# termuxinator/html5-canvas-raytracer

Measured on AMD Instinct MI355X. Metric: Mpixel/s, higher is better.
Workload: dtype f64; 1 GPU; cfg3: h8 scene (8 spheres, 2 lights, depth 3, supersample 1) at 3840x2160; SCENE, CAMERA AND LAUNCH TABLE RESIDENT (a static frame rendered again and again: cold_frame / new_camera_every_step are the other cases); one launch per frame; kernel=fma

## Files before the change

html5-canvas-raytracer_amd/csrc/rt_kernel_trace.h:

```cpp

#define RT_PIN() asm volatile("")
#define RT_ROOT(TCA, DISC)                                                                    \
        const double thc_ = rt_sqrt_nn<REFRACT>(DISC);                                                 \
        const double t0_ = (TCA) - thc_, t1_ = (TCA) + thc_;                                  \
        const bool in_ = (t0_ < eps);                                                         \
        const double t_ = in_ ? t1_ : t0_;
#define RT_CAND(IDX, TCA, DISC)                                                               \
      if (!((DISC) < 0.0)) {                                                                  \
        RT_PIN();                                                                             \
        RT_ROOT(TCA, DISC)                                                                    \
        const bool closer_ = (t_ < ht) && !(t_ < eps);              \
        ht = closer_ ? t_ : ht;                                                               \
        hcode = closer_ ? ((int)(2u * (IDX)) + (in_ ? 1 : 0)) : hcode;                        \
      }
#define RT_GENERIC(IDX, G)                                                                    \
      {                                                                                       \
        const v3 Lv_ = mk((G).ox - p.x, (G).oy - p.y, (G).oz - p.z);                          \
        const double tca_ = dot(d, Lv_);                                                      \
        const double disc_ = (G).r2 - (dot(Lv_, Lv_) - tca_ * tca_);                          \
        RT_CAND(IDX, tca_, disc_)                                                             \
      }
#define RT_ANCHORED_DISC(G)                                                                   \
        const double tca_ = d.x * (G).ox + d.y * (G).oy + d.z * (G).oz;                       \
        const double disc_ = __builtin_fma(tca_, tca_, -(G).r2);
#define RT_ANCHORED(IDX, G)                                                                   \
      {                                                                                       \
        RT_ANCHORED_DISC(G)                                                                   \
        RT_CAND(IDX, tca_, disc_)                                                             \
      }

#if !RT_STRICT
__device__ __forceinline__ float rt_q_of(float qp, float x, float c, float rp_over_r) {
  const float ic = __builtin_amdgcn_rcpf(fmaxf(c, 1e-30f));
  return fminf(ic * (qp * (6.f * x + rp_over_r) + x + 0.5f * x * x) + x, 1e30f);
}
__device__ __forceinline__ int rt_lvl(int lv) { return lv & 255; }
#define RT_Q_GET(L_) __builtin_bit_cast(float, (uint32_t)(L_) & 0xffff0000u)
__device__ __forceinline__ int rt_q_put(int lv, float q) { return (int)(((uint32_t)lv & 0xffffu) | ((__builtin_bit_cast(uint32_t, q) + 0xffffu) & 0xffff0000u)); }
__device__ __forceinline__ float rt_r_get(int lv) { return __builtin_bit_cast(float, ((uint32_t)lv & 0xff00u) << 15); }
__device__ __forceinline__ int rt_r_put(int lv, float r) { return (int)(((uint32_t)lv & 0xffff00ffu) | ((((__builtin_bit_cast(uint32_t, r) >> 23) + 1u) & 255u) << 8)); }
constexpr float RT_Q_FLAT = 4096.f;
#define RT_Q_OF(QP, T, INVR, C, RP) rt_q_of((QP), (T) * (INVR), (C), (RP) * (INVR))
#else
__device__ __forceinline__ int rt_lvl(int lv) { return lv; }
#endif

#if !RT_STRICT
#define RT_XY_INDEX(XU, XV, FU, FV)                                                                                \
          const unsigned long long su = __builtin_bit_cast(unsigned long long, (XU) + 6442450944.0), sv = __builtin_bit_cast(unsigned long long, (XV) + 6442450944.0);   \
          uint32_t iu = __builtin_amdgcn_alignbit((uint32_t)(su >> 32), (uint32_t)su, 20u) ^ 0x80000000u;        \
          uint32_t iv = __builtin_amdgcn_alignbit((uint32_t)(sv >> 32), (uint32_t)sv, 20u) ^ 0x80000000u;       \
           \
          const bool near_ = (min(((uint32_t)su + 1u) & 0xfffffu, ((uint32_t)sv + 1u) & 0xfffffu) <= 2u);           \
           \
          if constexpr (UNI) { if (__ballot(near_) != 0ull) return false; }                                    \
          if (!UNI && near_) {                                                                                  \
            RT_PIN();                                                                                             \
            iu = (uint32_t)(XU); iv = (uint32_t)(XV);                    \
            const rt_launch __attribute__((address_space(4))) *K = rt_cold_args();                                \
             \
            float q_here = RT_Q_GET(level);                                                                        \
            if (rt_lvl(level) == 0 && q_here == 0.f) {                   \
              const float ex = (float)(h.x - K->cam_origin[0]), ey = (float)(h.y - K->cam_origin[1]), ez = (float)(h.z - K->cam_origin[2]);   \
              q_here = RT_Q_OF(0.f, __builtin_sqrtf(ex * ex + ey * ey + ez * ez), (float)m.inv_r, __builtin_fabsf((float)dot(d, n)), 0.f);       \
            }                                                                                                     \
            double tol = (K->mark_flags & RT_MARK_ALL) ? 2.0 : K->flag_tol * (double)fmaxf(1.f, q_here * (1.f / RT_Q_FLAT));   \
                          \
            if ((K->mark_flags & (RT_MARK_WEIGHT | RT_MARK_ALL)) == RT_MARK_WEIGHT) {                              \
              double S_ = map_valid ? acc[0] : 1.0;                                                               \
              if constexpr (FOLD_FORWARD && REFRACT) for (int i_ = 0; i_ < sp; i_++) S_ *= (parked[i_].map_valid ? parked[i_].S : 1.0) * parked[i_].a3;   \
              if (__builtin_fabs(S_) * 510.0 < 0.9) tol = -1.0;                                                    \
            }                                                                                                     \
             \
            const bool zf = !(K->mark_flags & RT_MARK_ZERO);                                                       \
            const bool bu = (zf && (FU) == 0.0 && (XU) == 0.0) || (__builtin_fabs((XU) - __builtin_rint(XU)) >= tol);    \
            const bool bv = (zf && (FV) == 0.0 && (XV) == 0.0) || (__builtin_fabs((XV) - __builtin_rint(XV)) >= tol);    \
            if (!(bu & bv)) {                                                                                      \
              uint32_t t3 = threadIdx.x;                                                                          \
              if constexpr (W1 && !GRID) t3 = rt_lane_again(); else                                               \
              asm volatile("" : "+v"(t3));                                                                        \
              rt_mark_append<SS2>(rt_pixel_of<SS2, W1>(L, t3));                                                        \
            }                                                                                                     \
          }
#endif

#if !RT_STRICT
#define RT_SDISC(G, TC, DISC)                                                                 \
            const double TC = -(sv.x * (G).ox + sv.y * (G).oy + sv.z * (G).oz);               \
            const double DISC = __builtin_fma(TC, TC, -(G).r2);
#define RT_SROOTS(TC, THC, T0, T1) const double T0 = llen - (TC + THC), T1 = llen - (TC - THC);
#else
#define RT_SDISC(G, TC, DISC)                                                                 \
            const v3 Lv_ = mk((G).ox - h.x, (G).oy - h.y, (G).oz - h.z);                      \
            const double TC = dot(sv, Lv_);                                                   \
            const double DISC = (G).r2 - (dot(Lv_, Lv_) - TC * TC);
#define RT_SROOTS(TC, THC, T0, T1) const double T0 = TC - THC, T1 = TC + THC;
#endif
#define RT_SHADOW(J, G)                                                                       \
            {                                                                                 \
              const bool other_ = ((int)(J) != hi);                                           \
              if (COUNT && other_ && !blocked) tests++;                                       \
              RT_SDISC(G, tc_, disc_)                                                         \
              if (other_ && !(disc_ < 0.0) && !blocked) {                                     \
                RT_PIN();                                                                     \
                const double thc_ = rt_sqrt_nn<REFRACT>(disc_);                                        \
                RT_SROOTS(tc_, thc_, t0_, t1_)                                                \
                const double t_ = (t0_ < eps) ? t1_ : t0_;                                    \
                if ((t_ < llen) && !(t_ < eps)) {                                             \
                  RT_PIN();                                                                   \
                  const double oa4_ = objs[J].albedo[4];                                      \
                  if (oa4_ != 0.0) li = rt_div(li, oa4_);    \
                  else { li = 0.0; blocked = true; }                                          \
                }                                                                             \
              }                                                                               \
            }
#define RT_SHADOW_U(J, G)                                                                     \
            {                                                                               \
              RT_SDISC(G, tc_, disc_)                                                       \
              if (((int)(J) != hi) && !(disc_ < 0.0)) {                                     \
                RT_PIN();                                                                   \
                const double thc_ = rt_sqrt_nn<REFRACT>(disc_);                                      \
                RT_SROOTS(tc_, thc_, t0_, t1_)                                              \
                const double t_ = (t0_ < eps) ? t1_ : t0_;                                  \
                if ((t_ < llen) && !(t_ < eps) && li != 0.0) {                              \
                  RT_PIN();                                                                 \
                  const double oa4_ = objs[J].albedo[4];                                    \
                  li = (oa4_ != 0.0) ? rt_div(li, oa4_) : 0.0;                              \
                }                                                                           \
              }                                                                             \
            }

template <bool REFRACT, bool COUNT, bool GRID, bool SS2, bool ITEM = false, bool W1 = false, bool UNI = false>
__device__ __forceinline__ bool trace_pixel(const rt_launch &L, const rt_mtl *mtl, const rt_texture_desc *tex,
                                            [[maybe_unused]] double *acc, [[maybe_unused]] const rt_geom *cull_lds, [[maybe_unused]] const rt_geom cull0, [[maybe_unused]] uint32_t lane,
                                            [[maybe_unused]] double blk_x0, [[maybe_unused]] double blk_x1, [[maybe_unused]] double blk_y0,
                                            [[maybe_unused]] double blk_y1, v3 p, v3 d, double rgb[3], uint32_t cnt[3],
                                            [[maybe_unused]] bool is_probe, [[maybe_unused]] uint32_t cand_host,
                                            [[maybe_unused]] uint32_t own_sx = 0u, [[maybe_unused]] uint32_t own_sy = 0u, [[maybe_unused]] uint32_t own_f = 0u) {
  static_assert(!UNI || (W1 && !REFRACT && !COUNT && !ITEM && !RT_STRICT), "uniform-material path: the one-wave-workgroup product kernels");
#ifdef RT_TESTING
  uint32_t probe_n = 0;
  double probe_li = 0.0;
#endif
  const sphere_kptr objs = (sphere_kptr)L.objects;
  const geom_kptr geom = (geom_kptr)L.geom;
  const uint32_t N = L.n_objects, NL = L.n_lights;
  const double eps = L.epsilon;
  const uint32_t NLOOP = L.n_loop;
  const uint32_t enc = L.enclosing;
  const bool cull_lds_on = (!RT_STRICT && !COUNT) ? (!GRID && !W1) : (L.cull_in_lds != 0u);
#if RT_STRICT
  constexpr bool FOLD_FORWARD = false;
#else
  constexpr bool FOLD_FORWARD = true;
#endif
  constexpr bool LEAN = !RT_STRICT && !REFRACT && !COUNT && !ITEM;
  [[maybe_unused]] frame<REFRACT> stack[FOLD_FORWARD ? 1 : RT_MAX_SEGS];
  [[maybe_unused]] park parked[(FOLD_FORWARD && REFRACT) ? RT_MAX_SEGS : 1];
  [[maybe_unused]] int sp = 0;
  [[maybe_unused]] bool map_valid = false;
  int level = 0;
  [[maybe_unused]] uint32_t tree_path = 1u;
#if defined(RT_TESTING) && defined(RT_ABLATE_BOUNCE)
  uint32_t segs_left = L.segs ? 1 : 0;
#else
  uint32_t segs_left = L.segs;
#endif
  double ret[3] = {0.0, 0.0, 0.0};
  constexpr bool PARK_RET = FOLD_FORWARD && W1 && !GRID && !REFRACT && !COUNT && !ITEM && !UNI;

  double ht = RT_INF; int hcode = -1;
  if constexpr (UNI) { if (segs_left == 0) return false; }
  if (segs_left != 0) {
        [[maybe_unused]] const geom_kptr ga = (geom_kptr)L.geom_cam;
#if !RT_STRICT
        if constexpr (UNI) {
          const uint32_t i = cand_host & 255u;
          const rt_geom g0 = rt_load_geom32(ga, i);
          typename rt_mtl_src<true>::type &mu = *rt_mtl_at<true>(mtl, i);
          if ((mu.albedo[3] > 0.0 && segs_left > 1) || rt_mtl_kind(mu) == RT_SAMPLER_STARS) return false;
          RT_ANCHORED_DISC(g0)
          const double t0_ = tca_ - rt_sqrt_nn<REFRACT>(disc_);
          const bool met_ = !(disc_ < 0.0) && (t0_ < ht) && !(t0_ < eps);
          if (__ballot(!met_) != 0ull) return false;
#if defined(RT_TESTING) && defined(RT_ABLATE_UNIFORM)
          rgb[0] = rgb[1] = rgb[2] = 0.0;
          return true;
#endif
          ht = t0_; hcode = (int)(2u * i);
        } else
        if (cand_host != 0u) {
          { const uint32_t i = cand_host & 255u; const rt_geom g0 = rt_load_geom32(ga, i); RT_ANCHORED(i, g0) }
          if (cand_host >= (2u << 16)) { const uint32_t i = (cand_host >> 8) & 255u; const rt_geom g0 = rt_load_geom32(ga, i); RT_ANCHORED(i, g0) }
        } else
#endif
        for (uint32_t base = 0; base < NLOOP; base += 64u) {
          const uint32_t j = base + lane;
          const uint32_t jj = j < NLOOP ? j : 0u;
          double c0 = cull0.ox, c1 = cull0.oy, c2 = cull0.oz, c3 = cull0.r2;
          if constexpr (ITEM) {
          } else if (cull_lds_on) {
            const rt_geom __attribute__((address_space(3))) *g = (const rt_geom __attribute__((address_space(3))) *)cull_lds + jj;
            c0 = g->ox; c1 = g->oy; c2 = g->oz; c3 = g->r2;
          } else if (base != 0u || (W1 && !GRID)) {
            const rt_geom __attribute__((address_space(1))) *g = (const rt_geom __attribute__((address_space(1))) *)L.cull + jj;
            c0 = g->ox; c1 = g->oy; c2 = g->oz; c3 = g->r2;
          }
          const rt_geom cr = rt_geom{c0, c1, c2, c3};
          unsigned long long m = __ballot(j < NLOOP) & __ballot(cr.ox * L.proj_d <= blk_x1) & __ballot(cr.oy * L.proj_d >= blk_x0) &
                                 __ballot(cr.oz * L.proj_d <= blk_y1) & __ballot(cr.r2 * L.proj_d >= blk_y0);
          if constexpr (ITEM) m = (NLOOP - base >= 64u) ? ~0ull : ((1ull << (NLOOP - base)) - 1ull);
          while (m) {
            const uint32_t i = base + (uint32_t)__builtin_ctzll(m);
            m &= m - 1ull;
#if RT_STRICT
            const rt_geom g0 = rt_load_geom32(geom, i);
            RT_GENERIC(i, g0)
#else
            const rt_geom g0 = rt_load_geom32(ga, i);
            RT_ANCHORED(i, g0)
#endif
          }
        }
  }
  bool searched = true;
  [[maybe_unused]] bool first_bounce = false;
#if !RT_STRICT
  if (!UNI && L.sky_fast && segs_left != 0 && __ballot(hcode >= 0) == 0ull) {
    if (COUNT) { cnt[0]++; cnt[2] += N; }
    rgb[0] = L.sky_rgb[0]; rgb[1] = L.sky_rgb[1]; rgb[2] = L.sky_rgb[2];
    return true;
  }
#endif

  if (segs_left != 0) {
    for (;;) {
      if constexpr (PARK_RET) ret[0] = ret[1] = ret[2] = 0.0;
      if (COUNT) cnt[0]++;
      if (!UNI && !searched) {
        bool scanned = false;
#if !RT_STRICT
        if constexpr (GRID) {
          if (rt_cold_args()->bounce_table != nullptr) {
            const uint32_t from = (uint32_t)(hcode >> 1);
            const double ax = __builtin_fabs(d.x), ay = __builtin_fabs(d.y), az = __builtin_fabs(d.z);
            const bool bx = (ax >= ay) && (ax >= az), by = !bx && (ay >= az);
            const double dm = bx ? d.x : (by ? d.y : d.z);
            const double du = bx ? d.y : d.x, dv = (bx || by) ? d.z : d.y;
            const double sc = (0.5 * RT_BGRID) * __builtin_amdgcn_rcp(__builtin_fabs(dm));
            const double fu = __builtin_fmin(__builtin_fmax(__builtin_fma(du, sc, 0.5 * RT_BGRID), 0.0), (double)(RT_BGRID - 1u));
            const double fv = __builtin_fmin(__builtin_fmax(__builtin_fma(dv, sc, 0.5 * RT_BGRID), 0.0), (double)(RT_BGRID - 1u));
            const uint32_t face = (bx ? 0u : (by ? 2u : 4u)) + ((dm < 0.0) ? 1u : 0u);
            const uint32_t key = from * RT_BCELLS + face * (RT_BGRID * RT_BGRID) + (uint32_t)fv * RT_BGRID + (uint32_t)fu;
            const uint32_t words = (NLOOP + 63u) >> 6;
            ht = RT_INF; hcode = -1;
            for (uint32_t wd = 0; wd < words; wd++) {
              unsigned long long cand = 0ull, todo = __ballot(true);
              uint32_t distinct = 0;
              while (todo) {
                const uint32_t k0 = (uint32_t)__builtin_amdgcn_readlane((int)key, (int)__builtin_ctzll(todo));
                cand |= rt_load_word32(rt_cold_args()->bounce_table, k0 * words + wd);
                todo &= ~__ballot(key == k0);
                if (++distinct == 16u && todo) {
                  cand = (wd + 1u == words && (NLOOP & 63u)) ? ((1ull << (NLOOP & 63u)) - 1ull) : ~0ull;
                  break;
                }
              }
              while (cand) {
                const uint32_t j = (wd << 6) + (uint32_t)__builtin_ctzll(cand);
                cand &= cand - 1ull;
                const rt_geom g0 = rt_load_geom32(geom, j);
                RT_GENERIC(j, g0)
              }
            }
            scanned = true;
          }
        }
#endif
#if !RT_STRICT
        if constexpr (!GRID && !REFRACT && !COUNT && !ITEM) {
          if (first_bounce) {
            uint32_t fb = rt_entry_first_bounce<W1>(L);
#ifdef RT_TESTING
            if (L.no_first_bounce) fb = 0u;
#endif
            if (fb >> 31) {
              ht = RT_INF; hcode = -1;
              uint32_t m = (fb >> RT_CELL_SHIFT) & ((1u << RT_FB_MAX_LOOP) - 1u);
              uint32_t sn = rt_entry_second_node<W1>(L);
#ifdef RT_TESTING
              if (L.no_second_node) sn = 0u;
              if ((sn & (RT_SN_SELF0 | RT_SN_SELF1)) && L.uniform_waves != nullptr && __builtin_ctzll(__ballot(true)) == (int)lane) atomicAdd(L.uniform_waves + 3, 1ull);
#endif
              if (sn & RT_SN_SELF0) m &= ~(1u << (fb & 255u));
              if (sn & RT_SN_SELF1) m &= ~(1u << ((fb >> 8) & 255u));
              while (m) {
                const uint32_t i = (uint32_t)__builtin_ctz(m);
                m &= m - 1u;
                const rt_geom g0 = rt_load_geom32(geom, i);
                RT_GENERIC(i, g0)
              }
              scanned = true;
#ifdef RT_TESTING
              if (L.uniform_waves != nullptr && __builtin_ctzll(__ballot(true)) == (int)lane) atomicAdd(L.uniform_waves + 2, 1ull);
#endif
            }
          }
        }
#endif
        if (!scanned) {
          ht = RT_INF; hcode = -1;
          uint32_t i = 0;
          for (; i + 2 <= NLOOP; i += 2) {
            const rt_geom_pair gp = rt_load_geom_pair32(geom, i);
            const rt_geom g0 = gp.a, g1 = gp.b;
            RT_GENERIC(i, g0) RT_GENERIC(i + 1, g1)
          }
          if (i < NLOOP) { const rt_geom g0 = rt_load_geom32(geom, i); RT_GENERIC(i, g0) }
        }
      }
      [[maybe_unused]] const bool primary_node = UNI || searched;
      first_bounce = searched;
      searched = false;
      if (!UNI && enc != ~0u && hcode < 0) {
        if (L.enclosing_flat) {
          ht = 1.0; hcode = (int)(2u * enc + 1u);
        } else {
          const rt_geom g0 = rt_load_geom32(geom, enc);
          RT_GENERIC(enc, g0)
        }
      }
      if (COUNT) cnt[2] += N;
      const int hi = UNI ? (int)(cand_host & 255u) : (hcode >> 1);
      const bool inside = (hcode & 1) != 0;
      bool descend = false;
#if defined(RT_TESTING) && defined(RT_ABLATE_SHADE)
      if (true) { ret[0] = ht; ret[1] = (double)hcode; ret[2] = 0.0; } else
#endif
      if (!UNI && hcode < 0) {
        { const auto &mc = RT_COLD(miss_color); ret[0] = mc[0]; ret[1] = mc[1]; ret[2] = mc[2]; }
#ifdef RT_TESTING
        if (is_probe && probe_n < RT_PROBE_NODES) {
          double *q = L.probe + (size_t)(probe_n++) * RT_PROBE_WORDS;
          for (uint32_t z = 0; z < RT_PROBE_WORDS; z++) q[z] = 0.0;
          q[0] = (double)(REFRACT ? tree_path : (1u << rt_lvl(level))); q[1] = -1.0; q[2] = ht; q[9] = d.x; q[10] = d.y; q[11] = d.z;
          q[17] = (double)segs_left; q[19] = p.x; q[20] = p.y; q[21] = p.z; q[23] = 1.0;
        }
#endif
      } else {
        typename rt_mtl_src<UNI>::type &m = *rt_mtl_at<UNI>(mtl, (uint32_t)hi);
        const v3 h = mk(p.x + d.x * ht, p.y + d.y * ht, p.z + d.z * ht);
#if RT_STRICT
        double nlen;
        const v3 n = unit(mk(h.x - m.origin[0], h.y - m.origin[1], h.z - m.origin[2]), &nlen);
#else
        const double inv_r = m.inv_r;
        const v3 n = mk((h.x - m.origin[0]) * inv_r, (h.y - m.origin[1]) * inv_r, (h.z - m.origin[2]) * inv_r);
#endif
        v3 l;
        if constexpr (UNI) l = n;
        else l = inside ? mk(-n.x, -n.y, -n.z) : n;
        double a0 = m.albedo[0];
        const double a1 = m.albedo[1], a2 = m.albedo[2];
        double a3 = m.albedo[3];
        const double a4 = REFRACT ? m.albedo[4] : 0.0;
#if !RT_STRICT && !defined(RT_ABLATE_QAMP)
        if (!UNI && (rt_lvl(level) != 0 || ((a3 > 0.0 || a4 > 0.0) && segs_left > 1))) {
          const float ir_ = (float)inv_r;
          const float q_ = RT_Q_OF(RT_Q_GET(level), (float)ht, ir_, __builtin_fabsf((float)dot(d, n)), rt_r_get(level));
          level = rt_q_put(level, q_);
          level = rt_r_put(level, __builtin_amdgcn_rcpf(ir_));
        }
#endif

        double col[3];
#if defined(RT_TESTING) && defined(RT_ABLATE_SAMPLER)
        const int kind = RT_SAMPLER_COLOR;
#else
        const int kind = rt_mtl_kind(m);
#endif
#if RT_STRICT
        if (kind == RT_SAMPLER_TEXTURE) {
          double t_at, t_as;
          rt_atan2_asin<REFRACT>(-n.z, -n.x, -n.y, &t_at, &t_as);
          const double u = RT_DIV_CONST(t_at, M_PI) / 2.0 + 0.5;
          const double v = RT_DIV_CONST(t_as, M_PI / 2.0) / 2.0 + 0.5;
          const rt_texture_desc td = rt_tex_desc<UNI>(tex, rt_mtl_texture(m));
          const double xd = ceil(u * (double)td.width) - 1.0, yd = ceil(v * (double)td.height) - 1.0;
          uint32_t xi = (xd > 0.0) ? (uint32_t)xd : 0u, yi = (yd > 0.0) ? (uint32_t)yd : 0u;
          xi = min(xi, td.width - 1u); yi = min(yi, td.height - 1u);
          const uint32_t texel = *(const uint32_t *)(L.texel_base + td.texels_offset + ((size_t)yi * td.width + xi) * 4u);
          col[0] = RT_DIV_CONST((double)(texel & 255u), 255.0); col[1] = RT_DIV_CONST((double)((texel >> 8) & 255u), 255.0);
          col[2] = RT_DIV_CONST((double)((texel >> 16) & 255u), 255.0);
          if (xd != xd || yd != yd) col[0] = col[1] = col[2] = __builtin_nan("");
        } else if (kind == RT_SAMPLER_CHECKER) {
          double t_at, t_as;
          rt_atan2_asin<REFRACT>(-n.y, -n.x, -n.z, &t_at, &t_as);
          const double u = RT_DIV_CONST(t_at, M_PI) / 2.0 + 0.5;
          const double v = RT_DIV_CONST(t_as, M_PI / 2.0) / 2.0 + 0.5;
          const int c = to_int32_bit0(u * m.c[6]) ^ to_int32_bit0(v * m.c[7]);
          col[0] = m.c[3 * c]; col[1] = m.c[3 * c + 1]; col[2] = m.c[3 * c + 2];
#else
        [[maybe_unused]] double t_at, t_as;
        [[maybe_unused]] const bool one_cell = UNI && !GRID && kind == RT_SAMPLER_CHECKER && (cand_host & (1u << 24)) != 0u;
        if (UNI && one_cell) {
          const uint32_t c3 = (cand_host >> 28) & 1u ? 3u : 0u;
          col[0] = m.c[c3]; col[1] = m.c[c3 + 1u]; col[2] = m.c[c3 + 2u];
        } else if (UNI && kind != RT_SAMPLER_TEXTURE && kind != RT_SAMPLER_CHECKER) {
          col[0] = m.c[0]; col[1] = m.c[1]; col[2] = m.c[2];
        } else {
        if constexpr (UNI) {
          const bool tx_ = (kind == RT_SAMPLER_TEXTURE);
          rt_atan2_asin<REFRACT>(tx_ ? -n.z : -n.y, -n.x, tx_ ? -n.y : -n.z, &t_at, &t_as);
        }
        if (kind == RT_SAMPLER_TEXTURE) {
          if constexpr (!UNI) rt_atan2_asin<REFRACT>(-n.z, -n.x, -n.y, &t_at, &t_as);
          const double u = RT_DIV_CONST(t_at, M_PI) / 2.0 + 0.5;
          const double v = RT_DIV_CONST(t_as, M_PI / 2.0) / 2.0 + 0.5;
          const rt_texture_desc td = rt_tex_desc<UNI>(tex, rt_mtl_texture(m));
          const double xu = u * (double)td.width, xv = v * (double)td.height;
          RT_XY_INDEX(xu, xv, 1.0, 1.0)
          const uint32_t xi = min(iu, td.width - 1u), yi = min(iv, td.height - 1u);
          const uint32_t texel = *(const uint32_t *)(rt_cold_args()->texel_base + td.texels_offset + ((size_t)yi * td.width + xi) * 4u);
          col[0] = RT_DIV_CONST((double)(texel & 255u), 255.0); col[1] = RT_DIV_CONST((double)((texel >> 8) & 255u), 255.0);
          col[2] = RT_DIV_CONST((double)((texel >> 16) & 255u), 255.0);
        } else if (kind == RT_SAMPLER_CHECKER) {
          if constexpr (!UNI) rt_atan2_asin<REFRACT>(-n.y, -n.x, -n.z, &t_at, &t_as);
          const double u = RT_DIV_CONST(t_at, M_PI) / 2.0 + 0.5;
          const double v = RT_DIV_CONST(t_as, M_PI / 2.0) / 2.0 + 0.5;
          const double xu = u * m.c[6], xv = v * m.c[7];
          RT_XY_INDEX(xu, xv, m.c[6], m.c[7])
          const int c = (int)((iu ^ iv) & 1u);
          if constexpr (UNI) {
            double k0 = m.c[0], k1 = m.c[1], k2 = m.c[2], k3 = m.c[3], k4 = m.c[4], k5 = m.c[5];
            asm volatile("" : "+s"(k0), "+s"(k1), "+s"(k2), "+s"(k3), "+s"(k4), "+s"(k5));
            col[0] = c ? k3 : k0; col[1] = c ? k4 : k1; col[2] = c ? k5 : k2;
          } else { col[0] = m.c[3 * c]; col[1] = m.c[3 * c + 1]; col[2] = m.c[3 * c + 2]; }
#endif
        } else if (!UNI && kind == RT_SAMPLER_STARS) {
          uint32_t sx = own_sx, sy = own_sy, f = own_f;
          if constexpr (!ITEM) {
            f = blockIdx.z;
            uint32_t t3 = threadIdx.x;
            if constexpr (W1 && !GRID) t3 = rt_lane_again(); else
            asm volatile("" : "+v"(t3));
            const rt_pixel P = rt_pixel_of<SS2, W1>(L, t3);
            sx = SS2 ? 2u * P.px + (P.sub & 1u) : P.px; sy = SS2 ? 2u * P.frow + (P.sub >> 1) : P.frow;
          }
          const unsigned long long pix = (unsigned long long)sy * (SS2 ? 2u * L.w : L.w) + sx;
          const uint32_t path = REFRACT ? tree_path : (1u << rt_lvl(level));
          const rt_launch __attribute__((address_space(4))) *K = rt_cold_args();
          const uint32_t mix = lowbias32(K->stars_seed + K->stars_step * f);
          double c = star_uniform((uint32_t)pix, (uint32_t)(pix >> 32), path, mix);
          c = (c >= m.c[6]) ? 0.0 : c * m.c[7];
          col[0] = col[1] = col[2] = c;
        } else { col[0] = m.c[0]; col[1] = m.c[1]; col[2] = m.c[2]; }
#if !RT_STRICT
        }
#endif

        if constexpr (FOLD_FORWARD && REFRACT) {
#pragma unroll
          for (int c = 0; c < 3; c++) acc[(10 + c) * RT_WG_THREADS] = col[c];
        }

        double diffuse = 0.0, specular = 0.0;
        [[maybe_unused]] double draw = 0.0, sraw = 0.0;
#if defined(RT_TESTING) && defined(RT_ABLATE_LIGHT)
        if (false) {
#else
        if (a1 > 0.0 || a2 > 0.0) {
#endif
          double li = RT_COLD(light_intensity);
#if !RT_STRICT
          [[maybe_unused]] uint32_t smask = ~0u;
          if constexpr (!COUNT) { if (primary_node) smask = rt_entry_shadow_masks<W1>(L); }
#endif
          for (uint32_t k = 0; k < NL; k++) {
            double llen;
            const double *lk = (const double *)((const char *)&L.lights[0][0] + (uint32_t)(k * 24u));
#if !RT_STRICT
            [[maybe_unused]] rt_geom_pair gp_first;
            if constexpr (!GRID && !COUNT) {
              [[maybe_unused]] const geom_kptr gl = (geom_kptr)L.geom_light;
              gp_first = rt_load_geom_pair32(gl, k * L.n_objects);
            }
#endif
            const v3 sraw = mk(lk[0] - h.x, lk[1] - h.y, lk[2] - h.z);
            const double lmag = dot(sraw, sraw);
#if RT_STRICT
            const v3 sv = unit(sraw, &llen);
#else
            const double inv_llen = rt_rsqrt_pos(lmag);
            llen = lmag * inv_llen;
            const v3 sv = mk(sraw.x * inv_llen, sraw.y * inv_llen, sraw.z * inv_llen);
#endif
            const double sdot = dot(sv, l);
#if RT_STRICT
            if (sdot <= 0.0) continue;
#else
            if (!(sdot > 0.0)) continue;
#endif
            if (COUNT) cnt[1]++;
            uint32_t tests = 0;
            bool blocked = false;
#if !RT_STRICT
            const geom_kptr gl = (geom_kptr)L.geom_light;
            const uint32_t glo = k * L.n_objects;
#else
            const geom_kptr gl = geom;
            const uint32_t glo = 0u;
#endif
#if defined(RT_TESTING) && defined(RT_ABLATE_SHADOW)
            const uint32_t NS = 0;
#elif defined(RT_TESTING) && defined(RT_ABLATE_SHADOW4)
            const uint32_t NS = NLOOP > 4u ? NLOOP - 4u : NLOOP;
#else
            const uint32_t NS = NLOOP;
#endif
#if !RT_STRICT
            bool no_occluder = false;
            if constexpr (!COUNT) no_occluder = primary_node && k < 2u && ((smask >> (16u * k)) & 0xffffu) == 0u;
            if (no_occluder) {
            } else
            if (GRID && rt_cold_args()->shadow_grid != nullptr && li != 0.0) {
              const void *const sgrid = rt_cold_args()->shadow_grid;
              const double __attribute__((address_space(4))) *gh = (const double __attribute__((address_space(4))) *)sgrid + 16u * k;
              const v3 vv = mk(-sraw.x, -sraw.y, -sraw.z);
              const double vx = gh[0] * vv.x + gh[1] * vv.y + gh[2] * vv.z, vy = gh[3] * vv.x + gh[4] * vv.y + gh[5] * vv.z;
              const double vz = gh[6] * vv.x + gh[7] * vv.y + gh[8] * vv.z;
              const double iz = rt_rcp(vz);
              const double fx = __builtin_fmin(__builtin_fmax((vx * iz - gh[9]) * gh[11], 0.0), (double)(RT_SGRID - 1));
              const double fy = __builtin_fmin(__builtin_fmax((vy * iz - gh[10]) * gh[12], 0.0), (double)(RT_SGRID - 1));
              const bool proj = (vz > 0.0) && (fx == fx) && (fy == fy);
              const uint32_t cell = proj ? (uint32_t)fy * RT_SGRID + (uint32_t)fx : (uint32_t)(RT_SGRID * RT_SGRID);
              const uint32_t words = (NLOOP + 63u) >> 6;
              const uint32_t cells_at = 16u * NL + k * (RT_SGRID * RT_SGRID + 1u) * words;
              for (uint32_t wd = 0; wd < words; wd++) {
                unsigned long long cand = 0ull, todo = __ballot(true);
                while (todo) {
                  const uint32_t c0 = (uint32_t)__builtin_amdgcn_readlane((int)cell, (int)__builtin_ctzll(todo));
                  cand |= rt_load_word32(sgrid, cells_at + c0 * words + wd);
                  todo &= ~__ballot(cell == c0);
                }
                while (cand) {
                  const uint32_t j = (wd << 6) + (uint32_t)__builtin_ctzll(cand);
                  cand &= cand - 1ull;
                  const rt_geom g0 = rt_load_geom32(gl, glo + j);
                  RT_SHADOW_U(j, g0)
                }
              }
            } else
#endif
            if (!COUNT) {
              if constexpr (UNI) RT_PIN();
              if (li != 0.0) {
                uint32_t j = 0;
#if !RT_STRICT
                [[maybe_unused]] uint32_t mk = ~0u;
                if constexpr (!GRID) { if (primary_node && k < 2u) mk = (smask >> (16u * k)) | 0xffff0000u; }
                if constexpr (!GRID) {
                  if (NS >= 2u) { if (mk & 3u) { const rt_geom g0 = gp_first.a, g1 = gp_first.b; RT_SHADOW_U(0u, g0) RT_SHADOW_U(1u, g1) } j = 2u; }
                }
#endif
                for (; j + 2 <= NS; j += 2) {
#if !RT_STRICT
                  if (!GRID && j < 31u && ((mk >> j) & 3u) == 0u) continue;
#endif
                  const rt_geom_pair gp = rt_load_geom_pair32(gl, glo + j);
                  const rt_geom g0 = gp.a, g1 = gp.b;
                  RT_SHADOW_U(j, g0) RT_SHADOW_U(j + 1, g1)
                }
#if !RT_STRICT
                if (j < NS && (GRID || j >= 32u || ((mk >> j) & 1u))) { const rt_geom g0 = rt_load_geom32(gl, glo + j); RT_SHADOW_U(j, g0) }
#else
                if (j < NS) { const rt_geom g0 = rt_load_geom32(gl, glo + j); RT_SHADOW_U(j, g0) }
#endif
              }
            } else
            if (COUNT || li != 0.0) {
              uint32_t j = 0;
              for (; j + 2 <= NS; j += 2) {
                const rt_geom g0 = rt_load_geom32(gl, glo + j), g1 = rt_load_geom32(gl, glo + j + 1);
                RT_SHADOW(j, g0) RT_SHADOW(j + 1, g1)
                if (blocked) break;
              }
              if (j < NS && !blocked) { const rt_geom g0 = rt_load_geom32(gl, glo + j); RT_SHADOW(j, g0) }
            }
            if (COUNT) cnt[2] += tests;
            if (li == 0.0) continue;
#if RT_STRICT
            diffuse += li * sdot / lmag;
#else
            diffuse += (li * sdot) * (inv_llen * inv_llen);
#endif
#if defined(RT_TESTING) && defined(RT_ABLATE_SPEC)
            if (false) {
#else
            if (a2 > 0.0) {
#endif
#if RT_STRICT
              double ql;
              const v3 q = unit(reflect(mk(-sv.x, -sv.y, -sv.z), l), &ql);
              const double spd = d.x * -q.x + d.y * -q.y + d.z * -q.z;
#else
              const double t2 = 2.0 * sdot;
              const v3 q = mk(__builtin_fma(l.x, t2, -sv.x), __builtin_fma(l.y, t2, -sv.y), __builtin_fma(l.z, t2, -sv.z));
              const double spd = -(d.x * q.x + d.y * q.y + d.z * q.z);
#endif
#if !RT_STRICT
              typename rt_mtl_src<UNI>::type *spec_m = &m;
              if constexpr (GRID && !REFRACT && !COUNT && !UNI) {
                uint32_t off_ = (uint32_t)hi * (uint32_t)sizeof(rt_mtl);
                asm volatile("" : "+v"(off_));
                spec_m = (const rt_mtl *)((const char *)mtl + off_);
              }
              const int32_t spec_n = spec_m->spec_n;
              if (spd > 0.0) specular += rt_pow_spec<UNI>(spd, spec_n, &spec_m->specular_exponent);
#else
              if (spd > 0.0) specular += rt_pow(spd, m.specular_exponent);
#endif
            }
          }
          if constexpr (UNI) {
            draw = diffuse; sraw = specular;
            diffuse = rt_min1_nn(diffuse) * a1;
            specular = rt_min1_nn(specular) * a2;
          } else {
          diffuse = min1(diffuse) * a1;
          specular = min1(specular) * a2;
          }
#ifdef RT_TESTING
          probe_li = li;
#endif
        }

        if constexpr (PARK_RET) {
          uint32_t hi2 = (uint32_t)hi;
          asm volatile("" : "+v"(hi2));
          const rt_mtl &m2 = *rt_mtl_at<false>(mtl, hi2);
          a0 = m2.albedo[0]; a3 = m2.albedo[3];
        }

#if RT_STRICT
        const v3 nq = n;
#else
        const v3 nq = inside ? mk(-l.x, -l.y, -l.z) : l;
#endif
        v3 r = mk(0, 0, 0); double rlen = 0.0;
#if !RT_STRICT
        if constexpr (LEAN) { if (!UNI && a3 > 0.0 && segs_left > 1) r = unit_go(reflect(d, l), &rlen); } else
#endif
        if (!UNI && a3 > 0.0 && segs_left > 1) r = unit(reflect(d, nq), &rlen);
        v3 f = mk(0, 0, 0); double flen = 0.0;
        if (REFRACT && a4 > 0.0 && segs_left > 1) {
          const double dn = dot(d, nq);
          double cosi = -((dn < -1.0) ? -1.0 : min1(dn));
          v3 nn = nq; double eta;
          if (cosi < 0.0) { cosi = -cosi; nn = mk(-nq.x, -nq.y, -nq.z); eta = m.refract_index; }
          else eta = rt_rcp(m.refract_index);
          const double k = 1.0 - eta * eta * (1.0 - cosi * cosi);
          if (k > 0.0) {
            const double q = eta * cosi - rt_sqrt(k);
            f = mk(d.x * eta + nn.x * q, d.y * eta + nn.y * q, d.z * eta + nn.z * q);
          } else f = reflect(d, nn);
          f = unit(f, &flen);
        }

        if constexpr (FOLD_FORWARD && REFRACT) {
#pragma unroll
          for (int c = 0; c < 3; c++) col[c] = acc[(10 + c) * RT_WG_THREADS];
        }
        const bool go_r = !UNI && (rlen != 0.0);
        const bool go_f = REFRACT && (flen != 0.0);
#ifdef RT_TESTING
        if (is_probe && probe_n < RT_PROBE_NODES) {
          double *q = L.probe + (size_t)(probe_n++) * RT_PROBE_WORDS;
          q[0] = (double)(REFRACT ? tree_path : (1u << rt_lvl(level))); q[1] = (double)hcode; q[2] = ht;
          q[3] = h.x; q[4] = h.y; q[5] = h.z; q[6] = n.x; q[7] = n.y; q[8] = n.z; q[9] = d.x; q[10] = d.y; q[11] = d.z;
          q[12] = col[0]; q[13] = col[1]; q[14] = col[2]; q[15] = diffuse; q[16] = specular; q[17] = (double)segs_left;
          q[18] = probe_li; q[19] = p.x; q[20] = p.y; q[21] = p.z; q[22] = (double)(go_r ? 1 : 0) + 2.0 * (go_f ? 1 : 0); q[23] = 1.0;
        }
#endif
        if (!go_r && !go_f) {
          if constexpr (UNI) {
            double x[3];
#pragma unroll
            for (int c = 0; c < 3; c++) x[c] = col[c] * diffuse + col[c] * specular;
            const double poison = (((draw + sraw) + x[0]) + x[1]) + x[2];
            if (__ballot(poison != poison) == 0ull) {
#pragma unroll
              for (int c = 0; c < 3; c++) ret[c] = rt_max_nn(col[c] * a0, rt_min1_nn(x[c]));
            } else {
#if defined(RT_TESTING) && defined(RT_ABLATE_LIGHT)
              const bool lit = false;
#else
              const bool lit = (a1 > 0.0 || a2 > 0.0);
#endif
              const double d2 = lit ? min1(draw) * a1 : 0.0, s2 = lit ? min1(sraw) * a2 : 0.0;
#pragma unroll
              for (int c = 0; c < 3; c++) ret[c] = maxa(col[c] * a0, min1(col[c] * d2 + col[c] * s2));
            }
          } else
#pragma unroll
          for (int c = 0; c < 3; c++) ret[c] = maxa(col[c] * a0, min1(col[c] * diffuse + col[c] * specular));
        } else if constexpr (FOLD_FORWARD) {
          const uint32_t T = W1 ? 64u : RT_WG_THREADS;
          double A[3], D[3];
#pragma unroll
          for (int c = 0; c < 3; c++) { A[c] = col[c] * a0; D[c] = col[c] * diffuse + col[c] * specular; }
          const bool via_f = REFRACT && !go_r;
          if (REFRACT && go_r && go_f) {
            park &pk = parked[sp++];
#pragma unroll
            for (int c = 0; c < 3; c++) { pk.amb[c] = A[c]; pk.ds[c] = D[c]; }
            pk.a3 = a3; pk.a4 = a4; pk.h[0] = h.x; pk.h[1] = h.y; pk.h[2] = h.z; pk.f[0] = f.x; pk.f[1] = f.y; pk.f[2] = f.z;
            pk.path = tree_path; pk.segs_left = segs_left; pk.level = level; pk.map_valid = map_valid; pk.hcode = hcode;
            if (map_valid) {
              pk.S = acc[0];
#pragma unroll
              for (int c = 0; c < 3; c++) { pk.O[c] = acc[(1 + c) * T]; pk.LO[c] = acc[(4 + c) * T]; pk.HI[c] = acc[(7 + c) * T]; }
            }
            map_valid = false;
            p = h; d = r; tree_path = 2u * tree_path;
          } else {
            const double coef = via_f ? a4 : a3;
            if (!map_valid) {
              acc[0] = coef;
#pragma unroll
              for (int c = 0; c < 3; c++) { acc[(1 + c) * T] = D[c]; acc[(4 + c) * T] = A[c]; acc[(7 + c) * T] = LEAN ? rt_max1_nn(A[c]) : __builtin_fmax(A[c], 1.0); }
            } else {
              const double S = acc[0];
#pragma unroll
              for (int c = 0; c < 3; c++) {
                const double O = acc[(1 + c) * T], LO = acc[(4 + c) * T], HI = acc[(7 + c) * T];
                if constexpr (LEAN) {
                  const double l2 = __builtin_fma(S, A[c], O), h2 = __builtin_fma(S, rt_max1_nn(A[c]), O);
                  acc[(1 + c) * T] = __builtin_fma(S, D[c], O);
                  acc[(4 + c) * T] = rt_max_nn(LO, rt_min_nn(HI, l2));
                  acc[(7 + c) * T] = rt_max_nn(LO, rt_min_nn(HI, h2));
                } else {
                const double l2 = __builtin_fma(S, A[c], O), h2 = __builtin_fma(S, __builtin_fmax(A[c], 1.0), O);
                acc[(1 + c) * T] = __builtin_fma(S, D[c], O);
                acc[(4 + c) * T] = __builtin_fmax(LO, __builtin_fmin(HI, l2));
                acc[(7 + c) * T] = __builtin_fmax(LO, __builtin_fmin(HI, h2));
                }
              }
              acc[0] = S * coef;
            }
            map_valid = true;
            p = h; d = via_f ? f : r; tree_path = 2u * tree_path + (via_f ? 1u : 0u);
          }
          level++; segs_left--;
          descend = true;
        } else {
          frame<REFRACT> &fr = stack[level];
#pragma unroll
          for (int c = 0; c < 3; c++) { fr.amb[c] = col[c] * a0; fr.ds[c] = col[c] * diffuse + col[c] * specular; }
          fr.a3 = a3;
          if constexpr (REFRACT) {
            fr.a4 = a4; fr.h[0] = h.x; fr.h[1] = h.y; fr.h[2] = h.z; fr.f[0] = f.x; fr.f[1] = f.y; fr.f[2] = f.z;
            fr.re[0] = fr.re[1] = fr.re[2] = 0.0;
            fr.has_f = go_f; fr.phase = go_r ? 0 : 1;
          }
          p = h; d = go_r ? r : f;
          tree_path = 2u * tree_path + (go_r ? 0u : 1u);
          level++; segs_left--;
          descend = true;
        }
      }
      if (descend) continue;

      if constexpr (FOLD_FORWARD) {
        const uint32_t T = W1 ? 64u : RT_WG_THREADS;
        if (map_valid) {
          const double S = acc[0];
#pragma unroll
          for (int c = 0; c < 3; c++) {
            if constexpr (LEAN) ret[c] = rt_max_nn(acc[(4 + c) * T], rt_min_nn(acc[(7 + c) * T], __builtin_fma(S, ret[c], acc[(1 + c) * T])));
            else ret[c] = __builtin_fmax(acc[(4 + c) * T], __builtin_fmin(acc[(7 + c) * T], __builtin_fma(S, ret[c], acc[(1 + c) * T])));
          }
        }
        bool resumed = false;
        if constexpr (REFRACT) {
          if (sp > 0) {
            const park &pk = parked[--sp];
            const double coef = pk.a4;
            if (!pk.map_valid) {
              acc[0] = coef;
#pragma unroll
              for (int c = 0; c < 3; c++) {
                acc[(1 + c) * T] = pk.ds[c] + ret[c] * pk.a3; acc[(4 + c) * T] = pk.amb[c]; acc[(7 + c) * T] = __builtin_fmax(pk.amb[c], 1.0);
              }
            } else {
              const double S = pk.S;
#pragma unroll
              for (int c = 0; c < 3; c++) {
                const double Dn = pk.ds[c] + ret[c] * pk.a3;
                const double l2 = __builtin_fma(S, pk.amb[c], pk.O[c]), h2 = __builtin_fma(S, __builtin_fmax(pk.amb[c], 1.0), pk.O[c]);
                acc[(1 + c) * T] = __builtin_fma(S, Dn, pk.O[c]);
                acc[(4 + c) * T] = __builtin_fmax(pk.LO[c], __builtin_fmin(pk.HI[c], l2));
                acc[(7 + c) * T] = __builtin_fmax(pk.LO[c], __builtin_fmin(pk.HI[c], h2));
              }
              acc[0] = S * coef;
            }
            map_valid = true;
            p = mk(pk.h[0], pk.h[1], pk.h[2]); d = mk(pk.f[0], pk.f[1], pk.f[2]);
            tree_path = 2u * pk.path + 1u; segs_left = pk.segs_left - 1u; level = pk.level + 1;
            hcode = pk.hcode;

            resumed = true;
          }
        }
        if (!resumed) {
          if constexpr (PARK_RET) {
#pragma unroll
            for (int c = 0; c < 3; c++) acc[(1 + c) * T] = ret[c];
            uint32_t fin = 1u;
            asm volatile("" : "+v"(fin));
            if (fin != 0u) break;
          } else break;
        }
      } else {
        bool resumed = false;
        while (level > 0) {
          level--; segs_left++; tree_path >>= 1;
          frame<REFRACT> &fr = stack[level];
          if constexpr (REFRACT) {
            if (fr.phase == 0) {
              fr.re[0] = ret[0] * fr.a3; fr.re[1] = ret[1] * fr.a3; fr.re[2] = ret[2] * fr.a3;
              if (fr.has_f) {
                fr.phase = 1;
                p = mk(fr.h[0], fr.h[1], fr.h[2]); d = mk(fr.f[0], fr.f[1], fr.f[2]);
                tree_path = 2u * tree_path + 1u;
                level++; segs_left--;
                resumed = true;
                break;
              }
#pragma unroll
              for (int c = 0; c < 3; c++) ret[c] = maxa(fr.amb[c], min1(fr.ds[c] + fr.re[c]));
            } else {
#pragma unroll
              for (int c = 0; c < 3; c++) ret[c] = maxa(fr.amb[c], min1(fr.ds[c] + fr.re[c] + ret[c] * fr.a4));
            }
          } else {
#pragma unroll
            for (int c = 0; c < 3; c++) ret[c] = maxa(fr.amb[c], min1(fr.ds[c] + ret[c] * fr.a3));
          }
        }
        if (!resumed) break;
      }
    }
    if constexpr (PARK_RET) {
#pragma unroll
      for (int c = 0; c < 3; c++) ret[c] = acc[(1 + c) * 64u];
    }
  }
  rgb[0] = ret[0]; rgb[1] = ret[1]; rgb[2] = ret[2];
  return true;
}

#undef RT_Q_GET
#undef RT_Q_OF
#undef RT_ROOT
#undef RT_CAND
#undef RT_GENERIC
#undef RT_ANCHORED_DISC
#undef RT_ANCHORED
#undef RT_XY_INDEX
#undef RT_SDISC
#undef RT_SROOTS
#undef RT_SHADOW
#undef RT_SHADOW_U
```

Baseline: 168,100 Mpixel/s.

## Derive bounce state from node counter and fold chain end inline in W1 lean path

Adds a per-pixel node counter in the lean non-grid path, so the searched, first-bounce and map-valid flags and the level test come from the counter rather than from mutable state. In the single-wave path, the forward-folded affine map is applied right where each terminal shade is computed (miss or opaque hit), and the loop breaks directly. This removes the park-and-reload of ret through LDS and the opaque asm barrier. The shadow-mask skip test is also simplified to a clamped shift. Together these aim to cut register pressure and control flow in the hot bounce loop. The risk is that the flag derivation must exactly match the old semantics for every bounce pattern.

```diff
diff --git a/html5-canvas-raytracer_amd/csrc/rt_kernel_trace.h b/html5-canvas-raytracer_amd/csrc/rt_kernel_trace.h
--- a/html5-canvas-raytracer_amd/csrc/rt_kernel_trace.h
+++ b/html5-canvas-raytracer_amd/csrc/rt_kernel_trace.h
@@ -130,6 +130,15 @@
               }                                                                             \
             }
 
+#define RT_CHAIN_END()                                                                                                          \
+        if constexpr (SIX_WAVES) {                                                                                              \
+          if (map_valid) {                                                                                                      \
+            const double S_ = acc[0];                                                                                           \
+            _Pragma("unroll")                                                                                                   \
+            for (int c = 0; c < 3; c++) ret[c] = rt_max_nn(acc[(4 + c) * 64u], rt_min_nn(acc[(7 + c) * 64u], __builtin_fma(S_, ret[c], acc[(1 + c) * 64u])));   \
+          }                                                                                                                     \
+        }
+
 template <bool REFRACT, bool COUNT, bool GRID, bool SS2, bool ITEM = false, bool W1 = false, bool UNI = false>
 __device__ __forceinline__ bool trace_pixel(const rt_launch &L, const rt_mtl *mtl, const rt_texture_desc *tex,
                                             [[maybe_unused]] double *acc, [[maybe_unused]] const rt_geom *cull_lds, [[maybe_unused]] const rt_geom cull0, [[maybe_unused]] uint32_t lane,
@@ -167,7 +176,9 @@
   uint32_t segs_left = L.segs;
 #endif
   double ret[3] = {0.0, 0.0, 0.0};
-  constexpr bool PARK_RET = FOLD_FORWARD && W1 && !GRID && !REFRACT && !COUNT && !ITEM && !UNI;
+  constexpr bool SIX_WAVES = FOLD_FORWARD && W1 && !GRID && !REFRACT && !COUNT && !ITEM && !UNI;
+  constexpr bool WAVE_NODE = LEAN && !GRID && !UNI;
+  [[maybe_unused]] uint32_t turn = 0u;
 
   double ht = RT_INF; int hcode = -1;
   if constexpr (UNI) { if (segs_left == 0) return false; }
@@ -235,7 +246,11 @@
 
   if (segs_left != 0) {
     for (;;) {
-      if constexpr (PARK_RET) ret[0] = ret[1] = ret[2] = 0.0;
+      [[maybe_unused]] const uint32_t node_no = turn;
+      if constexpr (WAVE_NODE) {
+        turn++;
+        searched = (node_no == 0u); first_bounce = (node_no == 1u); map_valid = (node_no != 0u);
+      }
       if (COUNT) cnt[0]++;
       if (!UNI && !searched) {
         bool scanned = false;
@@ -320,8 +335,10 @@
         }
       }
       [[maybe_unused]] const bool primary_node = UNI || searched;
+      if constexpr (!WAVE_NODE) {
       first_bounce = searched;
       searched = false;
+      }
       if (!UNI && enc != ~0u && hcode < 0) {
         if (L.enclosing_flat) {
           ht = 1.0; hcode = (int)(2u * enc + 1u);
@@ -335,7 +352,7 @@
       const bool inside = (hcode & 1) != 0;
       bool descend = false;
 #if defined(RT_TESTING) && defined(RT_ABLATE_SHADE)
-      if (true) { ret[0] = ht; ret[1] = (double)hcode; ret[2] = 0.0; } else
+      if (true) { ret[0] = ht; ret[1] = (double)hcode; ret[2] = 0.0; RT_CHAIN_END() } else
 #endif
       if (!UNI && hcode < 0) {
         { const auto &mc = RT_COLD(miss_color); ret[0] = mc[0]; ret[1] = mc[1]; ret[2] = mc[2]; }
@@ -347,6 +364,7 @@
           q[17] = (double)segs_left; q[19] = p.x; q[20] = p.y; q[21] = p.z; q[23] = 1.0;
         }
 #endif
+        RT_CHAIN_END()
       } else {
         typename rt_mtl_src<UNI>::type &m = *rt_mtl_at<UNI>(mtl, (uint32_t)hi);
         const v3 h = mk(p.x + d.x * ht, p.y + d.y * ht, p.z + d.z * ht);
@@ -365,7 +383,7 @@
         double a3 = m.albedo[3];
         const double a4 = REFRACT ? m.albedo[4] : 0.0;
 #if !RT_STRICT && !defined(RT_ABLATE_QAMP)
-        if (!UNI && (rt_lvl(level) != 0 || ((a3 > 0.0 || a4 > 0.0) && segs_left > 1))) {
+        if (!UNI && ((WAVE_NODE ? node_no != 0u : rt_lvl(level) != 0) || ((a3 > 0.0 || a4 > 0.0) && segs_left > 1))) {
           const float ir_ = (float)inv_r;
           const float q_ = RT_Q_OF(RT_Q_GET(level), (float)ht, ir_, __builtin_fabsf((float)dot(d, n)), rt_r_get(level));
           level = rt_q_put(level, q_);
@@ -565,6 +583,7 @@
 #endif
                 for (; j + 2 <= NS; j += 2) {
 #if !RT_STRICT
+                  if constexpr (WAVE_NODE) { if (((mk >> (j < 30u ? j : 30u)) & 3u) == 0u) continue; } else
                   if (!GRID && j < 31u && ((mk >> j) & 3u) == 0u) continue;
 #endif
                   const rt_geom_pair gp = rt_load_geom_pair32(gl, glo + j);
@@ -635,7 +654,7 @@
 #endif
         }
 
-        if constexpr (PARK_RET) {
+        if constexpr (SIX_WAVES) {
           uint32_t hi2 = (uint32_t)hi;
           asm volatile("" : "+v"(hi2));
           const rt_mtl &m2 = *rt_mtl_at<false>(mtl, hi2);
@@ -701,9 +720,11 @@
 #pragma unroll
               for (int c = 0; c < 3; c++) ret[c] = maxa(col[c] * a0, min1(col[c] * d2 + col[c] * s2));
             }
-          } else
+          } else {
 #pragma unroll
           for (int c = 0; c < 3; c++) ret[c] = maxa(col[c] * a0, min1(col[c] * diffuse + col[c] * specular));
+          RT_CHAIN_END()
+          }
         } else if constexpr (FOLD_FORWARD) {
           const uint32_t T = W1 ? 64u : RT_WG_THREADS;
           double A[3], D[3];
@@ -748,7 +769,7 @@
               }
               acc[0] = S * coef;
             }
-            map_valid = true;
+            if constexpr (!WAVE_NODE) map_valid = true;
             p = h; d = via_f ? f : r; tree_path = 2u * tree_path + (via_f ? 1u : 0u);
           }
           level++; segs_left--;
@@ -771,7 +792,8 @@
       }
       if (descend) continue;
 
-      if constexpr (FOLD_FORWARD) {
+      if constexpr (SIX_WAVES) break;
+      else if constexpr (FOLD_FORWARD) {
         const uint32_t T = W1 ? 64u : RT_WG_THREADS;
         if (map_valid) {
           const double S = acc[0];
@@ -812,15 +834,7 @@
             resumed = true;
           }
         }
-        if (!resumed) {
-          if constexpr (PARK_RET) {
-#pragma unroll
-            for (int c = 0; c < 3; c++) acc[(1 + c) * T] = ret[c];
-            uint32_t fin = 1u;
-            asm volatile("" : "+v"(fin));
-            if (fin != 0u) break;
-          } else break;
-        }
+        if (!resumed) break;
       } else {
         bool resumed = false;
         while (level > 0) {
@@ -851,10 +865,6 @@
         if (!resumed) break;
       }
     }
-    if constexpr (PARK_RET) {
-#pragma unroll
-      for (int c = 0; c < 3; c++) ret[c] = acc[(1 + c) * 64u];
-    }
   }
   rgb[0] = ret[0]; rgb[1] = ret[1]; rgb[2] = ret[2];
   return true;
@@ -872,3 +882,4 @@
 #undef RT_SROOTS
 #undef RT_SHADOW
 #undef RT_SHADOW_U
+#undef RT_CHAIN_END
```

New measurement: 171,000 Mpixel/s (median of 6 runs). 1.02x the previous value.
